# JohnLonginotto/uq

Hardware: NVIDIA B200
Metric: fastq_to_uq_encode_reads_per_s (higher is better)
Workload: dtype u8

## Files before the change

### uq_b200/csrc/common.cuh

```cuda
#pragma once
#include <cuda_runtime.h>
#include <stdint.h>
#include <stdio.h>
#include <string.h>
#include <string>
#include <vector>
#include <map>
#include "../../include/uqb200.h"

#define UQB_SM_COUNT 148

struct uqb_timer_rec { const char* name; cudaEvent_t a, b; uint64_t bytes; };
struct uqb_timer_tot { uint64_t launches = 0; double ms = 0; uint64_t bytes = 0; };

struct uqb_arena {
    unsigned long long base = 0;
    uint64_t reserved = 0;
    uint64_t mapped = 0;
    uint64_t granularity = 0;
    std::map<uint64_t, uint64_t> free_by_off;
    std::map<uint64_t, uint64_t> used;
    std::vector<unsigned long long> handles;
    std::vector<std::pair<uint64_t, uint64_t>> chunks;
};
// ... 106 lines not shown
static inline unsigned uqb_grid(uqb_ctx* ctx, uint64_t n, unsigned per_block, unsigned waves = 8) {
    uint64_t need = (n + per_block - 1) / per_block;
    uint64_t cap = (uint64_t)ctx->sm_count * waves;
    if (need < 1) need = 1;
    return (unsigned)(need < cap ? need : cap);
}

#ifdef __CUDACC__
__device__ __forceinline__ unsigned lane_id() { return threadIdx.x & 31u; }

__device__ __forceinline__ uint64_t load_be64(const uint8_t* p, uint32_t avail) {
    uint64_t v = 0;
#pragma unroll
    for (int i = 0; i < 8; i++) {
        uint64_t b = (uint32_t)i < avail ? (uint64_t)__ldg(p + i) : 0ull;
        v = (v << 8) | b;
    }
    return v;
}

__device__ __forceinline__ void atomic_min_i64(int64_t* addr, int64_t v) {
    atomicMin((long long*)addr, (long long)v);
}
__device__ __forceinline__ void atomic_max_i64(int64_t* addr, int64_t v) {
    atomicMax((long long*)addr, (long long)v);
}
#endif

#define UQB_SPLIT_TILE (256 * 64)
int uqb_split_count_tiles(uqb_ctx* ctx, const uint8_t* d, uint64_t n_end, uint64_t tile0, uint64_t ntiles, uint32_t* counts);
int uqb_split_write_tiles(uqb_ctx* ctx, const uint8_t* d, uint64_t n_end, uint64_t tile0, uint64_t ntiles, uint64_t line_base,
                          const uint64_t* bases, uint64_t* line_off);
int uqb_split_set_first(uqb_ctx* ctx, uint64_t* line_off);
int uqb_copy_stream(uqb_ctx* ctx, cudaStream_t* out);
int uqb_names_release(uqb_ctx* ctx, uqb_fastq* fq);

int uqb_scan_u32(uqb_ctx* ctx, const uint32_t* d_in, uint32_t* d_out, uint64_t n, uint32_t* d_total);
int uqb_scan_u32_to_u64(uqb_ctx* ctx, const uint32_t* d_in, uint64_t* d_out, uint64_t n, uint64_t* d_total);

struct uqb_sortbuf {
    uint64_t* key[2] = {nullptr, nullptr};
    uint32_t* aux[2] = {nullptr, nullptr};
    uint32_t* val[2] = {nullptr, nullptr};
    int cur = 0;
    uint64_t cap = 0;
};
int uqb_sortbuf_alloc(uqb_ctx* ctx, uqb_sortbuf* sb, uint64_t n, bool with_aux);
int uqb_sortbuf_free(uqb_ctx* ctx, uqb_sortbuf* sb);
int uqb_radix_sort(uqb_ctx* ctx, uqb_sortbuf* sb, uint64_t n, bool use_aux, const uint64_t* key_first = nullptr);
int uqb_scatter_pairs_u32(uqb_ctx* ctx, const uint32_t* idx, const uint32_t* val, uint64_t n, uint32_t* out);

int uqb_sort_rows_impl(uqb_ctx* ctx, const uint8_t* rows, uint64_t n, uint32_t width,
                       uint32_t** d_perm, uint32_t** d_gid_sorted, uint64_t* n_unique, const uint64_t* key0 = nullptr,
                       uint64_t** sorted_keys = nullptr);
```

### uq_b200/csrc/sort.cu

```cuda
#include "common.cuh"

#define ST 256

__global__ void __launch_bounds__(ST) k_chunk0_keys(const uint8_t* __restrict__ rows, uint64_t n, uint32_t width,
                                                   uint64_t* __restrict__ key, uint32_t* __restrict__ val) {
    uint64_t i = (uint64_t)blockIdx.x * ST + threadIdx.x;
    if (i >= n) return;
    key[i] = load_be64(rows + i * width, width < 8 ? width : 8);
    val[i] = (uint32_t)i;
}

#define SORT_ZOFF_MIN_WIDTH 256
__global__ void __launch_bounds__(ST) k_leading_zero_bytes(const uint8_t* __restrict__ rows, uint64_t n, uint32_t width,
                                                          uint32_t* __restrict__ zoff) {
    const unsigned lane = threadIdx.x & 31u;
    const uint64_t wstride = (uint64_t)gridDim.x * (ST / 32);
    for (uint64_t i = (uint64_t)blockIdx.x * (ST / 32) + (threadIdx.x >> 5); i < n; i += wstride) {
        const uint8_t* row = rows + i * width;
        uint32_t z = width;
        const uint32_t head = (uint32_t)((16u - ((uintptr_t)row & 15u)) & 15u);
        for (uint32_t b0 = 0; b0 < head && b0 < width && z == width; b0 += 32) {
            const uint32_t b = b0 + lane;
            const bool nz = b < head && b < width && row[b] != 0;
            const unsigned m = __ballot_sync(0xffffffffu, nz);
            if (m) z = b0 + (__ffs(m) - 1);
        }
        for (uint32_t b0 = head; b0 < width && z == width; b0 += 512) {
            const uint32_t b = b0 + lane * 16;
            uint32_t first = 16;
            if (b + 16 <= width) {
                const uint4 v = __ldg(reinterpret_cast<const uint4*>(row + b));
                if (v.x) first = (__ffs(v.x) - 1) >> 3;
                else if (v.y) first = 4 + ((__ffs(v.y) - 1) >> 3);
                else if (v.z) first = 8 + ((__ffs(v.z) - 1) >> 3);
                else if (v.w) first = 12 + ((__ffs(v.w) - 1) >> 3);
            } else if (b < width) {
                for (uint32_t k = 0; k < width - b; k++) if (row[b + k] != 0) { first = k; break; }
            }
            const unsigned m = __ballot_sync(0xffffffffu, first < 16);
            if (m) {
                const int src = __ffs(m) - 1;
                z = b0 + src * 16 + __shfl_sync(0xffffffffu, first, src);
            }
        }
        if (lane == 0) zoff[i] = z;
    }
}

__global__ void __launch_bounds__(ST) k_chunk0_keys_z(const uint8_t* __restrict__ rows, uint64_t n, uint32_t width, const uint32_t* __restrict__ zoff,
                                                     uint64_t* __restrict__ key, uint32_t* __restrict__ aux, uint32_t* __restrict__ val) {
    uint64_t i = (uint64_t)blockIdx.x * ST + threadIdx.x;
    if (i >= n) return;
    const uint32_t z = zoff[i], sig = width - z;
    key[i] = load_be64(rows + i * width + z, sig < 8 ? sig : 8);
    aux[i] = sig;
    val[i] = (uint32_t)i;
}

__global__ void __launch_bounds__(ST) k_mark_heads(const uint64_t* __restrict__ key, const uint32_t* __restrict__ aux, uint64_t n,
                                                  uint32_t* __restrict__ head) {
    uint64_t p = (uint64_t)blockIdx.x * ST + threadIdx.x;
    if (p >= n) return;
    head[p] = (p == 0 || key[p] != key[p - 1] || (aux && aux[p] != aux[p - 1])) ? 1u : 0u;
}

#define GLCP_EQUAL 0xFFFFFFFFu
__global__ void __launch_bounds__(ST) k_headpos(const uint32_t* __restrict__ head, const uint32_t* __restrict__ excl, uint64_t n,
                                               uint32_t* __restrict__ headpos, uint32_t* __restrict__ glcp) {
    uint64_t p = (uint64_t)blockIdx.x * ST + threadIdx.x;
    if (p >= n) return;
    if (head[p]) { headpos[excl[p]] = (uint32_t)p; glcp[excl[p]] = GLCP_EQUAL; }
    if (p == n - 1) headpos[excl[p] + head[p]] = (uint32_t)n;
}

template <int SUB>
__global__ void __launch_bounds__(ST) k_group_lcp(const uint8_t* __restrict__ rows, uint32_t width, uint32_t off, const uint32_t* __restrict__ zoff,
                                                 const uint32_t* __restrict__ perm, const uint32_t* __restrict__ head,
                                                 const uint32_t* __restrict__ excl, const uint32_t* __restrict__ headpos,
                                                 const uint8_t* __restrict__ done, uint64_t n, uint32_t* __restrict__ glcp) {
    constexpr uint32_t NP = 32u / SUB;
    constexpr int UN = 4;
    const unsigned lane = threadIdx.x & 31u, sg = lane / SUB, sl = lane % SUB;
    const uint64_t nblk = (n + 31) / 32, wstride = (uint64_t)gridDim.x * (ST / 32);
    for (uint64_t blk = (uint64_t)blockIdx.x * (ST / 32) + (threadIdx.x >> 5); blk < nblk; blk += wstride) {
        const uint64_t p = blk * 32 + lane;
        uint32_t ra = 0, rb = 0, g = 0, z = 0;
        bool live = false;
        if (p < n && !head[p] && !done[p]) {
            live = true;
            g = excl[p] - 1;
            ra = perm[p];
            rb = perm[headpos[g]];
            if (zoff) z = zoff[ra];
        }
        unsigned todo = __ballot_sync(0xffffffffu, live);
        if (!todo) continue;
        uint32_t mine = GLCP_EQUAL;
        for (uint32_t j0 = 0; j0 < 32; j0 += NP * UN) {
            if (!((todo >> j0) & ((NP * UN >= 32) ? 0xffffffffu : ((1u << (NP * UN)) - 1u)))) continue;
            uint32_t res[UN];
#pragma unroll
            for (int u = 0; u < UN; u++) res[u] = GLCP_EQUAL;
            uint32_t a_r[UN], b_r[UN], zz[UN];
            bool lv[UN];
#pragma unroll
            for (int u = 0; u < UN; u++) {
                const uint32_t j = j0 + u * NP + sg;
                a_r[u] = __shfl_sync(0xffffffffu, ra, j & 31u);
                b_r[u] = __shfl_sync(0xffffffffu, rb, j & 31u);
                zz[u] = __shfl_sync(0xffffffffu, z, j & 31u);
                lv[u] = j < 32u && ((todo >> (j & 31u)) & 1u);
            }
            const uint32_t maxrem = width - off;
            for (uint32_t w0 = 0; 4u * w0 < maxrem; w0 += SUB) {
                const uint32_t wd = w0 + sl;
                uint32_t xa[UN], xb[UN];
// ... 171 lines not shown
                        const uint32_t a = __shfl_sync(0xffffffffu, ord, pp & 31u);
                        int cc = 0;
#pragma unroll
                        for (int t = 0; t < TRIPS; t++) {
                            const uint32_t x = (pv && wvalid[t]) ? srows[a * pitch + t * SUB + sl] : y[t];
                            const unsigned ne = (__ballot_sync(0xffffffffu, x != y[t]) >> (sg * SUB)) & SUBMASK;
                            const unsigned lt = (__ballot_sync(0xffffffffu, x < y[t]) >> (sg * SUB)) & SUBMASK;
                            if (cc == 0 && ne) cc = ((lt >> (__ffs((int)ne) - 1)) & 1u) ? -1 : 1;
                        }
                        if (NP == 1) {
                            if (lane == q0) c = cc;
                        } else {
                            const int got = __shfl_sync(0xffffffffu, cc, ((lane - q0) * SUB) & 31u);
                            if (lane >= q0 && lane < q0 + NP && lane < hi) c = got;
                        }
                    }
                }
                have_c = false;
                const bool inr = lane >= lo && lane < hi;
                const unsigned less = __ballot_sync(0xffffffffu, inr && c < 0);
                const unsigned eq = __ballot_sync(0xffffffffu, inr && c == 0);
                const uint32_t nl = __popc(less), neq = __popc(eq);
                const uint32_t e0 = lo + nl, h0 = e0 + neq;
                if (nl | (hi - h0)) {
                    const unsigned gt = ((hi < 32u ? (1u << hi) : 0u) - (1u << lo)) & ~(less | eq);
                    uint32_t np = lane;
                    if (inr) np = c < 0 ? lo + __popc(less & ltm) : (c == 0 ? e0 + __popc(eq & ltm) : h0 + __popc(gt & ltm));
                    sord[np] = ord;
                    __syncwarp();
                    ord = sord[lane];
                    __syncwarp();
                }
                B |= 1u << e0;
                if (h0 < hi) B |= 1u << h0;
                R |= (uint32_t)((1ull << h0) - (1ull << e0));
                if (nl == 1u) R |= 1u << lo;
                if (hi - h0 == 1u) R |= 1u << h0;
            }
            const uint32_t rfin = __shfl_sync(0xffffffffu, r, ord & 31u);
            if (lane < sz) {
                perm[s + lane] = rfin;
                if (lane > 0) head[s + lane] = (B >> lane) & 1u;
                done[s + lane] = 1;
            }
            __syncwarp();
        }
    }
#pragma unroll
    for (int o = 16; o > 0; o >>= 1) my_large += __shfl_xor_sync(0xffffffffu, my_large, o);
    if (lane == 0 && my_large) atomicAdd(large_rows, my_large);
}

#define SGP_CHUNK 2048
template <int SUB>
__global__ void __launch_bounds__(ST) k_small_groups_packed(const uint8_t* __restrict__ rows, uint32_t width, uint32_t off,
                                                           uint32_t* __restrict__ perm, const uint32_t* __restrict__ head, uint32_t* __restrict__ head_out,
                                                           uint8_t* __restrict__ done, uint64_t n, uint32_t pitch,
                                                           unsigned long long* __restrict__ large_rows) {
    extern __shared__ uint32_t sg_smem[];
    constexpr uint32_t NP = 32u / SUB;
    constexpr uint32_t SUBMASK = SUB == 32 ? 0xffffffffu : ((1u << (SUB & 31)) - 1u);
    const unsigned lane = threadIdx.x & 31u, w = threadIdx.x >> 5;
    const unsigned sg = lane / SUB, sl = lane % SUB;
    uint32_t* srows = sg_smem + (size_t)w * (32 * pitch);
    const uint32_t rem = width - off;
    const bool wvalid = sl < pitch;
    const uint32_t nvalid = wvalid ? rem - 4u * sl : 0u;
    const uint32_t tailmask = nvalid >= 4u ? 0xffffffffu : (nvalid ? 0xffffffffu << ((4u - nvalid) * 8u) : 0u);
    const uint64_t nchunks = (n + SGP_CHUNK - 1) / SGP_CHUNK, warps_total = (uint64_t)gridDim.x * (ST / 32);
    unsigned long long my_large = 0;
    for (uint64_t ck = (uint64_t)blockIdx.x * (ST / 32) + w; ck < nchunks; ck += warps_total) {
        const uint64_t c0 = ck * SGP_CHUNK, c1 = (c0 + SGP_CHUNK < n) ? c0 + SGP_CHUNK : n;
        uint64_t cur = c0;
        while (cur < c1) {
            const unsigned hb = __ballot_sync(0xffffffffu, cur + lane < n ? head[cur + lane] != 0u : true);
            if (hb) { cur += (unsigned)__ffs((int)hb) - 1u; break; }
            cur += 32;
        }
        while (cur < c1) {
            const uint32_t r_spec = cur + lane < n ? perm[cur + lane] : 0u;
            const unsigned h1 = __ballot_sync(0xffffffffu, cur + lane < n ? head[cur + lane] != 0u : true);
            const unsigned h2 = __ballot_sync(0xffffffffu, cur + 32 + lane < n ? head[cur + 32 + lane] != 0u : true);
            const unsigned hi = (h1 >> 1) | (h2 << 31);
            if (!hi) {
                uint64_t nxt = c1;
                if (h2 >> 1) nxt = cur + 32 + ((unsigned)__ffs((int)(h2 >> 1)));
                else {
                    for (uint64_t q = cur + 64; q < c1; q += 32) {
                        const unsigned hb = __ballot_sync(0xffffffffu, q + lane < n ? head[q + lane] != 0u : true);
                        if (hb) { nxt = q + (unsigned)__ffs((int)hb) - 1u; break; }
                    }
                }
                if (lane == 0) my_large += 33;
                cur = nxt;
                continue;
            }
            const uint32_t cnt = 32u - (uint32_t)__clz((int)hi);
            const unsigned live = cnt == 32u ? 0xffffffffu : ((1u << cnt) - 1u);
            const unsigned hm = h1 & live;
            if (hm == live) { cur += cnt; continue; }
            const uint32_t r = lane < cnt ? r_spec : 0u;
            const unsigned upto = (2u << lane) - 1u;
            const uint32_t gs = 31u - (uint32_t)__clz((int)(hm & upto));
            const unsigned above = hm & ~upto;
            const uint32_t ge = above ? (uint32_t)__ffs((int)above) - 1u : cnt;
            const bool multi = lane < cnt && ge - gs > 1u;
            const unsigned need = __ballot_sync(0xffffffffu, multi);
#pragma unroll 4
            for (uint32_t j0 = 0; j0 < cnt; j0 += NP) {
                const uint32_t j = j0 + sg;
                const uint32_t rj = __shfl_sync(0xffffffffu, r, j & 31u);
                if (j < cnt && ((need >> j) & 1u) && wvalid) {
                    const uint64_t A = (uint64_t)(uintptr_t)rows + (uint64_t)rj * width + off;
                    const uint32_t ph = (uint32_t)A & 3u;
                    const uint32_t* base = reinterpret_cast<const uint32_t*>(A - ph) + sl;
                    const uint32_t lo = __ldg(base), hi2 = __ldg(base + 1);
                    srows[j * pitch + sl] = __byte_perm(__funnelshift_r(lo, hi2, ph * 8u), 0u, 0x0123) & tailmask;
                }
            }
            __syncwarp();
            const uint32_t maxsz = __reduce_max_sync(0xffffffffu, multi ? ge - gs : 0u);
            unsigned dmask = 0;
            for (uint32_t j0 = 0; j0 < cnt; j0 += NP) {
                const uint32_t j = j0 + sg;
                const uint32_t sj = __shfl_sync(0xffffffffu, gs, j & 31u);
                bool ne = false;
                if (j < cnt && ((need >> j) & 1u) && wvalid) ne = srows[j * pitch + sl] != srows[sj * pitch + sl];
                const unsigned b = __ballot_sync(0xffffffffu, ne);
#pragma unroll
                for (uint32_t s2 = 0; s2 < NP; s2++) if (lane == j0 + s2) dmask = (b >> (s2 * SUB)) & SUBMASK;
            }
            uint32_t rank = 0;
            bool eq_before = false;
            for (uint32_t t = 0; t < maxsz; t++) {
                const uint32_t i = gs + t;
                const bool act = multi && i < ge && i != lane;
                const unsigned di = __shfl_sync(0xffffffffu, dmask, act ? i : lane);
                if (act) {
                    unsigned m = di | dmask;
                    int c = 0;
                    while (m) {
                        const uint32_t wd = (uint32_t)__ffs((int)m) - 1u;
                        m &= m - 1u;
                        const uint32_t a = srows[i * pitch + wd], b = srows[lane * pitch + wd];
                        if (a != b) { c = a < b ? -1 : 1; break; }
                    }
                    if (c < 0 || (c == 0 && i < lane)) rank++;
                    if (c == 0 && i < lane) eq_before = true;
                }
            }
            __syncwarp();
            if (multi) {
                perm[cur + gs + rank] = r;
                if (rank > 0) head_out[cur + gs + rank] = eq_before ? 0u : 1u;
                done[cur + lane] = 1;
            }
            cur += cnt;
        }
    }
    if (lane == 0 && my_large) atomicAdd(large_rows, my_large);
}

__global__ void __launch_bounds__(ST) k_small_groups_gmem(const uint8_t* __restrict__ rows, uint32_t width, uint32_t off,
                                                         const uint32_t* __restrict__ zoff, uint32_t* __restrict__ perm, uint32_t* __restrict__ head, uint8_t* __restrict__ done,
                                                         const uint32_t* __restrict__ headpos, const uint32_t* __restrict__ d_ngroups,
                                                         unsigned long long* __restrict__ large_rows) {
    const unsigned lane = threadIdx.x & 31u, w = threadIdx.x >> 5;
    const uint32_t G = *d_ngroups;
    const uint64_t warps_total = (uint64_t)gridDim.x * (ST / 32);
    unsigned long long my_large = 0;
    for (uint64_t g0 = ((uint64_t)blockIdx.x * (ST / 32) + w) * 32; g0 < G; g0 += warps_total * 32) {
        const uint64_t g = g0 + lane;
        uint32_t start = 0, size = 0;
        if (g < G) { start = headpos[g]; size = headpos[g + 1] - start; }
        const bool fin = size < 2 || done[start];
        if (size > SG_MAX && !fin) my_large += size;
        unsigned need = __ballot_sync(0xffffffffu, size <= SG_MAX && !fin);
        while (need) {
            const int src = __ffs(need) - 1;
            need &= need - 1;
            const uint32_t s = __shfl_sync(0xffffffffu, start, src), sz = __shfl_sync(0xffffffffu, size, src);
            const uint32_t r = lane < sz ? perm[s + lane] : 0u;
            const uint32_t z = __shfl_sync(0xffffffffu, (zoff && lane < sz) ? zoff[r] : 0u, 0);
            const uint32_t rem = z + off < width ? width - z - off : 0u;
            uint32_t rank = 0;
            bool eq_before = false;
            for (uint32_t j = 0; j < sz; j++) {
                const uint32_t rj = __shfl_sync(0xffffffffu, r, j);
                if (lane < sz && j != lane) {
                    int c = 0;
                    const uint8_t* pa = rows + (uint64_t)rj * width + z + off;
                    const uint8_t* pb = rows + (uint64_t)r * width + z + off;
                    for (uint32_t i = 0; i < rem; i++) {
                        const unsigned a = __ldg(pa + i), b = __ldg(pb + i);
                        if (a != b) { c = a < b ? -1 : 1; break; }
                    }
                    if (c < 0 || (c == 0 && j < lane)) rank++;
                    if (c == 0 && j < lane) eq_before = true;
                }
            }
            __syncwarp();
            if (lane < sz) {
                perm[s + rank] = r;
                if (rank > 0) head[s + rank] = eq_before ? 0u : 1u;
                done[s + lane] = 1;
            }
            __syncwarp();
        }
    }
#pragma unroll
    for (int o = 16; o > 0; o >>= 1) my_large += __shfl_xor_sync(0xffffffffu, my_large, o);
    if (lane == 0 && my_large) atomicAdd(large_rows, my_large);
}

__global__ void __launch_bounds__(ST) k_compact_active(const uint8_t* __restrict__ rows, uint32_t width, const uint32_t* __restrict__ glcp,
                                                      const uint32_t* __restrict__ zoff, const uint32_t* __restrict__ act, const uint32_t* __restrict__ apos,
                                                      const uint32_t* __restrict__ head, const uint32_t* __restrict__ excl,
                                                      const uint32_t* __restrict__ perm, uint64_t n, uint32_t* __restrict__ pos_list,
                                                      uint64_t* __restrict__ key, uint32_t* __restrict__ aux, uint32_t* __restrict__ val) {
    uint64_t p = (uint64_t)blockIdx.x * ST + threadIdx.x;
    if (p >= n || !act[p]) return;
    uint32_t j = apos[p];
    uint32_t row = perm[p];
    pos_list[j] = (uint32_t)p;
    const uint32_t z = zoff ? zoff[row] : 0u;
    const uint32_t g = excl[p] + head[p] - 1;
    const uint32_t off = glcp[g];
    const uint32_t rem = z + off < width ? width - z - off : 0u;
    key[j] = load_be64(rows + (uint64_t)row * width + z + off, rem < 8 ? rem : 8);
    aux[j] = g;
    val[j] = row;
}

__global__ void __launch_bounds__(ST) k_write_back(const uint64_t* __restrict__ key, const uint32_t* __restrict__ aux,
                                                  const uint32_t* __restrict__ val, const uint32_t* __restrict__ pos_list, uint64_t m,
                                                  uint32_t* __restrict__ perm, uint32_t* __restrict__ head) {
    uint64_t j = (uint64_t)blockIdx.x * ST + threadIdx.x;
    if (j >= m) return;
    uint32_t p = pos_list[j];
    perm[p] = val[j];
    head[p] = (j == 0 || aux[j] != aux[j - 1] || key[j] != key[j - 1]) ? 1u : 0u;
}

__global__ void __launch_bounds__(ST) k_gid_from_scan(const uint32_t* __restrict__ head, uint32_t* __restrict__ excl_inout, uint64_t n) {
    uint64_t p = (uint64_t)blockIdx.x * ST + threadIdx.x;
    if (p >= n) return;
    excl_inout[p] = excl_inout[p] + head[p] - 1;
}

__global__ void __launch_bounds__(ST) k_iota_zero(uint32_t* __restrict__ perm, uint32_t* __restrict__ gid, uint64_t n) {
    uint64_t p = (uint64_t)blockIdx.x * ST + threadIdx.x;
    if (p >= n) return;
    perm[p] = (uint32_t)p;
    gid[p] = 0;
}

int uqb_sort_rows_impl(uqb_ctx* ctx, const uint8_t* rows, uint64_t n, uint32_t width,
                       uint32_t** d_perm, uint32_t** d_gid_sorted, uint64_t* n_unique, const uint64_t* key0, uint64_t** sorted_keys) {
    *d_perm = nullptr; *d_gid_sorted = nullptr; *n_unique = 0;
    if (sorted_keys) *sorted_keys = nullptr;
    if (n >= (1ull << 32)) return uqb_fail(ctx, "sort_rows: %llu rows exceed the 32-bit index range", (unsigned long long)n);
    uint32_t *perm = nullptr, *head, *excl;
    UQB_TRY(uqb_dalloc_t(ctx, &excl, n + 16));
    if (n == 0 || width == 0) UQB_TRY(uqb_dalloc_t(ctx, &perm, n + 16));
    if (n == 0) { *d_perm = perm; *d_gid_sorted = excl; return 0; }
    const unsigned nb = uqb_blocks(n, ST);
    if (width == 0) {
        UQB_LAUNCH(k_iota_zero, nb, ST, 0, perm, excl, n);
        *d_perm = perm; *d_gid_sorted = excl; *n_unique = 1;
        return 0;
    }
    UQB_TRY(uqb_dalloc_t(ctx, &head, n));
    uint32_t* d_tot;
    UQB_TRY(uqb_dalloc_t(ctx, &d_tot, 2));

    uint32_t* zoff = nullptr;
    if (width > SORT_ZOFF_MIN_WIDTH) {
        UQB_TRY(uqb_dalloc_t(ctx, &zoff, n));
        UQB_LAUNCH_B(n * 4, k_leading_zero_bytes, uqb_grid(ctx, n, ST / 32, 16), ST, 0, rows, n, width, zoff);
    }
    {
        uqb_sortbuf sb;
        UQB_TRY(uqb_sortbuf_alloc(ctx, &sb, n, zoff != nullptr));
        const uint64_t* kf = (!zoff && width >= 8) ? key0 : nullptr;
        if (zoff) UQB_LAUNCH_B(n * 24, k_chunk0_keys_z, nb, ST, 0, rows, n, width, zoff, sb.key[0], sb.aux[0], sb.val[0]);
        else if (!kf) UQB_LAUNCH_B(n * ((width < 8 ? width : 8) + 12), k_chunk0_keys, nb, ST, 0, rows, n, width, sb.key[0], sb.val[0]);
        UQB_TRY(uqb_radix_sort(ctx, &sb, n, zoff != nullptr, kf));
        UQB_LAUNCH(k_mark_heads, nb, ST, 0, sb.key[sb.cur], zoff ? sb.aux[sb.cur] : (const uint32_t*)nullptr, n, head);
        perm = sb.val[sb.cur];
        sb.val[sb.cur] = nullptr;
        if (sorted_keys && width <= 8 && !zoff) { *sorted_keys = sb.key[sb.cur]; sb.key[sb.cur] = nullptr; }
        UQB_TRY(uqb_sortbuf_free(ctx, &sb));
    }
    if (width > 8) {
        const uint32_t off = 8;
        uint32_t *headpos, *glcp, *act = nullptr, *apos = nullptr;
        uint8_t* done;
        unsigned long long* d_large;
        UQB_TRY(uqb_dalloc_t(ctx, &headpos, n + 1));
        UQB_TRY(uqb_dalloc_t(ctx, &glcp, n));
        UQB_TRY(uqb_dalloc_t(ctx, &done, n));
        UQB_TRY(uqb_dalloc_t(ctx, &d_large, 1));
        UQB_CUDA(cudaMemsetAsync(done, 0, n, ctx->stream));
        const uint32_t max_rounds = (width + 7) / 8 + 1;
        bool finished = false;
        if (width - off <= 128 && !zoff) {
            const uint32_t rem = width - off, pitch = (rem + 3) / 4;
            uint32_t* head2;
            UQB_TRY(uqb_dalloc_t(ctx, &head2, n));
            UQB_CUDA(cudaMemcpyAsync(head2, head, n * 4, cudaMemcpyDeviceToDevice, ctx->stream));
            UQB_CUDA(cudaMemsetAsync(d_large, 0, 8, ctx->stream));
            const size_t smem = (size_t)(ST / 32) * 32 * pitch * 4;
            const unsigned grid = uqb_grid(ctx, (n + SGP_CHUNK - 1) / SGP_CHUNK, ST / 32, 16);
            const uint64_t ab = n * ((uint64_t)rem + 13);
            if (pitch <= 8) {
                auto k_small_groups_packed_8 = k_small_groups_packed<8>;
                UQB_LAUNCH_B(ab, k_small_groups_packed_8, grid, ST, smem, rows, width, off, perm, head, head2, done, n, pitch, d_large);
            } else if (pitch <= 16) {
                auto k_small_groups_packed_16 = k_small_groups_packed<16>;
                UQB_LAUNCH_B(ab, k_small_groups_packed_16, grid, ST, smem, rows, width, off, perm, head, head2, done, n, pitch, d_large);
            } else {
                auto k_small_groups_packed_32 = k_small_groups_packed<32>;
                UQB_LAUNCH_B(ab, k_small_groups_packed_32, grid, ST, smem, rows, width, off, perm, head, head2, done, n, pitch, d_large);
            }
            UQB_TRY(uqb_dfree(ctx, head, n * 4));
            head = head2;
            unsigned long long large = 0;
            UQB_TRY(uqb_readback(ctx, &large, d_large, 8));
            finished = large == 0;
        }
        for (uint32_t round = 0; round < max_rounds && !finished; round++) {
            UQB_TRY(uqb_scan_u32(ctx, head, excl, n, d_tot));
            UQB_LAUNCH(k_headpos, nb, ST, 0, head, excl, n, headpos, glcp);
            const uint32_t rem = width - off;
            UQB_CUDA(cudaMemsetAsync(d_large, 0, 8, ctx->stream));
            const unsigned sg_grid = uqb_grid(ctx, n, ST, 16);
            if (rem <= SG_STAGE_BYTES && !zoff) {
                const uint32_t pitch = (rem + 3) / 4;
                const size_t smem = (size_t)(ST / 32) * (SG_MAX * pitch + 64) * 4;
                if (pitch <= 8) {
                    auto k_small_groups_8 = k_small_groups<8, 1>;
                    UQB_LAUNCH(k_small_groups_8, sg_grid, ST, smem, rows, width, off, perm, head, done, headpos, d_tot, pitch, d_large);
                } else if (pitch <= 16) {
                    auto k_small_groups_16 = k_small_groups<16, 1>;
                    UQB_LAUNCH(k_small_groups_16, sg_grid, ST, smem, rows, width, off, perm, head, done, headpos, d_tot, pitch, d_large);
                } else if (pitch <= 32) {
                    auto k_small_groups_32 = k_small_groups<32, 1>;
                    UQB_CUDA(cudaFuncSetAttribute(k_small_groups_32, cudaFuncAttributeMaxDynamicSharedMemorySize, (int)smem));
                    UQB_LAUNCH(k_small_groups_32, sg_grid, ST, smem, rows, width, off, perm, head, done, headpos, d_tot, pitch, d_large);
                } else {
                    auto k_small_groups_64 = k_small_groups<32, 2>;
                    UQB_CUDA(cudaFuncSetAttribute(k_small_groups_64, cudaFuncAttributeMaxDynamicSharedMemorySize, (int)smem));
                    UQB_LAUNCH(k_small_groups_64, sg_grid, ST, smem, rows, width, off, perm, head, done, headpos, d_tot, pitch, d_large);
                }
            } else {
                UQB_LAUNCH(k_small_groups_gmem, sg_grid, ST, 0, rows, width, off, zoff, perm, head, done, headpos, d_tot, d_large);
            }
            unsigned long long large = 0;
            UQB_TRY(uqb_readback(ctx, &large, d_large, 8));
            if (large == 0) break;
            const uint64_t ab_lcp = n * ((uint64_t)rem + 16);
            if (rem <= 32) {
                auto k_group_lcp_8 = k_group_lcp<8>;
                UQB_LAUNCH_B(ab_lcp, k_group_lcp_8, uqb_grid(ctx, n, ST, 16), ST, 0, rows, width, off, zoff, perm, head, excl, headpos, done, n, glcp);
            } else {
                auto k_group_lcp_32 = k_group_lcp<32>;
                UQB_LAUNCH_B(ab_lcp, k_group_lcp_32, uqb_grid(ctx, n, ST, 16), ST, 0, rows, width, off, zoff, perm, head, excl, headpos, done, n, glcp);
            }
            if (!act) {
                UQB_TRY(uqb_dalloc_t(ctx, &act, n));
                UQB_TRY(uqb_dalloc_t(ctx, &apos, n));
            }
            UQB_LAUNCH(k_active_flags, nb, ST, 0, head, excl, glcp, done, n, act);
            UQB_TRY(uqb_scan_u32(ctx, act, apos, n, d_tot + 1));
            uint32_t tot[2];
            UQB_TRY(uqb_readback(ctx, tot, d_tot, 8));
            const uint64_t m = tot[1];
            if (m == 0) break;
            uqb_sortbuf sb;
            uint32_t* pos_list;
            UQB_TRY(uqb_sortbuf_alloc(ctx, &sb, m, true));
            UQB_TRY(uqb_dalloc_t(ctx, &pos_list, m));
            UQB_LAUNCH_B(n * 8 + m * 32, k_compact_active, nb, ST, 0, rows, width, glcp, zoff, act, apos, head, excl, perm, n, pos_list, sb.key[0], sb.aux[0], sb.val[0]);
            UQB_TRY(uqb_radix_sort(ctx, &sb, m, true));
            UQB_LAUNCH_B(m * 28, k_write_back, uqb_blocks(m, ST), ST, 0, sb.key[sb.cur], sb.aux[sb.cur], sb.val[sb.cur], pos_list, m, perm, head);
            UQB_TRY(uqb_dfree(ctx, pos_list, m * 4));
            UQB_TRY(uqb_sortbuf_free(ctx, &sb));
        }
        UQB_TRY(uqb_dfree(ctx, headpos, (n + 1) * 4));
        UQB_TRY(uqb_dfree(ctx, glcp, n * 4));
        if (act) { UQB_TRY(uqb_dfree(ctx, act, n * 4)); UQB_TRY(uqb_dfree(ctx, apos, n * 4)); }
        UQB_TRY(uqb_dfree(ctx, done, n));
        UQB_TRY(uqb_dfree(ctx, d_large, 8));
    }
    if (zoff) UQB_TRY(uqb_dfree(ctx, zoff, n * 4));
    UQB_TRY(uqb_scan_u32(ctx, head, excl, n, d_tot));
    UQB_LAUNCH(k_gid_from_scan, nb, ST, 0, head, excl, n);
    uint32_t u;
    UQB_TRY(uqb_readback(ctx, &u, d_tot, 4));
    UQB_TRY(uqb_dfree(ctx, d_tot, 8));
    UQB_TRY(uqb_dfree(ctx, head, n * 4));
    *d_perm = perm;
    *d_gid_sorted = excl;
    *n_unique = u;
    return 0;
}

__global__ void __launch_bounds__(ST) k_scatter_key(const uint32_t* __restrict__ perm, const uint32_t* __restrict__ gid, uint64_t n,
                                                   uint32_t* __restrict__ key) {
    uint64_t p = (uint64_t)blockIdx.x * ST + threadIdx.x;
    if (p >= n) return;
    key[perm[p]] = gid[p];
}

static int scatter_key(uqb_ctx* ctx, const uint32_t* perm, const uint32_t* gid, uint64_t n, uint32_t* key) {
    if (n == 0) return 0;
    const uint32_t wshift = 23;
    if (n <= (3ull << wshift)) {
        UQB_LAUNCH_B(n * 12, k_scatter_key, uqb_blocks(n, ST), ST, 0, perm, gid, n, key);
        return 0;
    }
    return uqb_scatter_pairs_u32(ctx, perm, gid, n, key);
}

__global__ void __launch_bounds__(ST) k_first_of_group(const uint32_t* __restrict__ perm, const uint32_t* __restrict__ gid, uint64_t n,
                                                      uint32_t* __restrict__ first_row) {
    uint64_t p = (uint64_t)blockIdx.x * ST + threadIdx.x;
    if (p >= n) return;
    if (p == 0 || gid[p] != gid[p - 1]) first_row[gid[p]] = perm[p];
}

__global__ void __launch_bounds__(ST) k_uniq_from_keys(const uint64_t* __restrict__ skey, const uint32_t* __restrict__ gid, uint64_t n,
                                                      uint32_t width, uint8_t* __restrict__ out) {
    for (uint64_t p = (uint64_t)blockIdx.x * ST + threadIdx.x; p < n; p += (uint64_t)gridDim.x * ST) {
        const uint32_t g = gid[p];
        if (p && gid[p - 1] == g) continue;
        const uint64_t k = skey[p];
        uint8_t* o = out + (uint64_t)g * width;
        for (uint32_t b = 0; b < width; b++) o[b] = (uint8_t)(k >> (56 - 8 * b));
    }
}

__global__ void __launch_bounds__(ST) k_gather_rows(const uint8_t* __restrict__ table, uint32_t width, const uint32_t* __restrict__ idx,
                                                   uint64_t nrows, uint8_t* __restrict__ out) {
    const unsigned lane = threadIdx.x & 31u;
    const uint64_t wstride = (uint64_t)gridDim.x * (ST / 32);
    for (uint64_t i = (uint64_t)blockIdx.x * (ST / 32) + (threadIdx.x >> 5); i < nrows; i += wstride) {
        const uint8_t* src = table + (uint64_t)__ldg(idx + i) * width;
        uint8_t* dst = out + i * width;
        for (uint32_t b = lane; b < width; b += 32) dst[b] = __ldg(src + b);
    }
}
// ... 44 lines not shown
    __shared__ __align__(16) uint8_t stage[ST * 16];
    const uint64_t nblk = (nrows + ST - 1) / ST;
    for (uint64_t blk = blockIdx.x; blk < nblk; blk += gridDim.x) {
        const uint64_t i0 = blk * ST, i = i0 + threadIdx.x;
        const uint32_t nr = (uint32_t)(nrows - i0 < ST ? nrows - i0 : ST);
        __syncthreads();
        if (i < nrows) {
            const uint8_t* s = table + (uint64_t)__ldg(idx + i) * width;
            for (uint32_t b = 0; b < width; b++) stage[threadIdx.x * width + b] = __ldg(s + b);
        }
        __syncthreads();
        const uint32_t total = nr * width;
        uint8_t* dst = out + i0 * width;
        for (uint32_t k = threadIdx.x; k < (total >> 2); k += ST) reinterpret_cast<uint32_t*>(dst)[k] = reinterpret_cast<const uint32_t*>(stage)[k];
        if (threadIdx.x < (total & 3u)) dst[(total & ~3u) + threadIdx.x] = stage[(total & ~3u) + threadIdx.x];
    }
}

template <typename T>
__global__ void __launch_bounds__(ST) k_gather_items(const T* __restrict__ table, const uint32_t* __restrict__ idx, uint64_t n, T* __restrict__ out) {
    for (uint64_t i = (uint64_t)blockIdx.x * ST + threadIdx.x; i < n; i += (uint64_t)gridDim.x * ST) out[i] = table[idx[i]];
}

static int gather_rows_impl(uqb_ctx* ctx, const void* table, uint32_t width, const uint32_t* idx, uint64_t n, void* out) {
    if (n == 0 || width == 0) return 0;
    const uint64_t ab = n * (2 * (uint64_t)width + 4);
    const unsigned g = uqb_grid(ctx, n, ST, 16);
    switch (width) {
        case 1: UQB_LAUNCH_B(ab, k_gather_items<uint8_t>, g, ST, 0, (const uint8_t*)table, idx, n, (uint8_t*)out); return 0;
        case 2: UQB_LAUNCH_B(ab, k_gather_items<uint16_t>, g, ST, 0, (const uint16_t*)table, idx, n, (uint16_t*)out); return 0;
        case 4: UQB_LAUNCH_B(ab, k_gather_items<uint32_t>, g, ST, 0, (const uint32_t*)table, idx, n, (uint32_t*)out); return 0;
        case 8: UQB_LAUNCH_B(ab, k_gather_items<uint64_t>, g, ST, 0, (const uint64_t*)table, idx, n, (uint64_t*)out); return 0;
    }
    if ((reinterpret_cast<uintptr_t>(out) & 3u) == 0) {
        if (width <= 16) {
            UQB_LAUNCH_B(ab, k_gather_narrow, uqb_grid(ctx, n, ST, 16), ST, 0, (const uint8_t*)table, width, idx, n, (uint8_t*)out);
            return 0;
        }
        if (width <= GR_MAXW) {
            UQB_LAUNCH_B(ab, k_gather_rows32, uqb_grid(ctx, n, ST, 16), ST, 0, (const uint8_t*)table, width, 128u / width, 128u % width, idx, n, (uint8_t*)out);
            return 0;
        }
    }
    UQB_LAUNCH_B(ab, k_gather_rows, uqb_grid(ctx, n, ST / 32, 16), ST, 0, (const uint8_t*)table, width, idx, n, (uint8_t*)out);
    return 0;
}

extern "C" int uqb_sort_rows(uqb_ctx* ctx, const uqb_array* table, uqb_array** perm, uqb_array** key,
                             uqb_array** key_sorted, uqb_array** uniq, uint64_t* n_unique) {
    uint32_t *d_perm, *d_gid;
    uint64_t u = 0;
    const uint64_t n = table->n;
    uint64_t* skeys = nullptr;
    UQB_TRY(uqb_sort_rows_impl(ctx, (const uint8_t*)table->d, n, table->width, &d_perm, &d_gid, &u, table->key0, uniq ? &skeys : nullptr));
    if (n_unique) *n_unique = u;
    const unsigned nb = uqb_blocks(n, ST);
    if (key) {
        UQB_TRY(uqb_new_array(ctx, n, 4, key));
        UQB_TRY(scatter_key(ctx, d_perm, d_gid, n, (uint32_t*)(*key)->d));
    }
    if (uniq) {
        UQB_TRY(uqb_new_array(ctx, u, table->width, uniq));
        if (skeys) {
            UQB_LAUNCH_B(n * 12 + u * table->width, k_uniq_from_keys, uqb_grid(ctx, n, ST, 16), ST, 0, skeys, d_gid, n, table->width, (uint8_t*)(*uniq)->d);
            UQB_TRY(uqb_dfree(ctx, skeys, n * 8));
        } else if (n && table->width) {
            uint32_t* first_row;
            UQB_TRY(uqb_dalloc_t(ctx, &first_row, u));
            UQB_LAUNCH(k_first_of_group, nb, ST, 0, d_perm, d_gid, n, first_row);
            UQB_TRY(gather_rows_impl(ctx, table->d, table->width, first_row, u, (*uniq)->d));
            UQB_TRY(uqb_dfree(ctx, first_row, u * 4));
        }
    }
    if (key_sorted) UQB_TRY(uqb_adopt_array(ctx, d_gid, n, 4, key_sorted));
    else UQB_TRY(uqb_dfree(ctx, d_gid, n * 4));
    if (perm) UQB_TRY(uqb_adopt_array(ctx, d_perm, n, 4, perm));
    else UQB_TRY(uqb_dfree(ctx, d_perm, n * 4));
    return 0;
}

extern "C" int uqb_gather_rows(uqb_ctx* ctx, const uqb_array* table, const uqb_array* perm, uqb_array** out) {
    if (perm->width != 4) return uqb_fail(ctx, "gather_rows: index array must be uint32");
    UQB_TRY(uqb_new_array(ctx, perm->n, table->width, out));
    UQB_TRY(gather_rows_impl(ctx, table->d, table->width, (const uint32_t*)perm->d, perm->n, (*out)->d));
    return 0;
}

template <typename T>
__global__ void __launch_bounds__(ST) k_narrow(const uint32_t* __restrict__ in, uint64_t n, T* __restrict__ out) {
    for (uint64_t i = (uint64_t)blockIdx.x * ST + threadIdx.x; i < n; i += (uint64_t)gridDim.x * ST) out[i] = (T)in[i];
}

extern "C" int uqb_narrow_u32(uqb_ctx* ctx, const uqb_array* a, uint32_t itemsize, uqb_array** out) {
    if (a->width != 4) return uqb_fail(ctx, "narrow: input must be uint32");
    UQB_TRY(uqb_new_array(ctx, a->n, itemsize, out));
    if (a->n == 0) return 0;
    unsigned g = uqb_grid(ctx, a->n, ST, 16);
    const uint32_t* in = (const uint32_t*)a->d;
    switch (itemsize) {
        case 1: UQB_LAUNCH(k_narrow<uint8_t>, g, ST, 0, in, a->n, (uint8_t*)(*out)->d); break;
        case 2: UQB_LAUNCH(k_narrow<uint16_t>, g, ST, 0, in, a->n, (uint16_t*)(*out)->d); break;
        case 4: UQB_LAUNCH(k_narrow<uint32_t>, g, ST, 0, in, a->n, (uint32_t*)(*out)->d); break;
        case 8: UQB_LAUNCH(k_narrow<uint64_t>, g, ST, 0, in, a->n, (uint64_t*)(*out)->d); break;
        default: return uqb_fail(ctx, "narrow: itemsize %u", itemsize);
    }
    return 0;
}

template <typename T>
__global__ void __launch_bounds__(ST) k_index_u32(const T* __restrict__ in, uint64_t n, uint64_t bound, uint32_t* __restrict__ out,
                                                 unsigned long long* __restrict__ first_bad) {
    unsigned long long bad = ~0ull;
    for (uint64_t i = (uint64_t)blockIdx.x * ST + threadIdx.x; i < n; i += (uint64_t)gridDim.x * ST) {
        const unsigned long long v = (unsigned long long)in[i];
// ... 368 lines not shown
```

Before: 775.9 million.

## Emit unique rows directly from the small-group finisher kernel into per-chunk slots

When unique rows are requested and width fits, the small-group sort finisher writes each distinct row (sorted key prefix plus staged tail bytes) into per-chunk slots. A prefix scan then compacts them into the output, replacing the separate first-of-group plus gather-rows pass. It also adds a group-count readback after head marking, which gates the path on duplication being at least two to one. The cost is extra shared memory, lower occupancy bounds, a slot buffer sized to n·width, and an added host sync.

```diff
diff --git a/uq_b200/csrc/common.cuh b/uq_b200/csrc/common.cuh
--- a/uq_b200/csrc/common.cuh
+++ b/uq_b200/csrc/common.cuh
@@ -182,4 +182,4 @@
 
 int uqb_sort_rows_impl(uqb_ctx* ctx, const uint8_t* rows, uint64_t n, uint32_t width,
                        uint32_t** d_perm, uint32_t** d_gid_sorted, uint64_t* n_unique, const uint64_t* key0 = nullptr,
-                       uint64_t** sorted_keys = nullptr);
+                       uint64_t** sorted_keys = nullptr, uqb_array** uniq = nullptr);
diff --git a/uq_b200/csrc/sort.cu b/uq_b200/csrc/sort.cu
--- a/uq_b200/csrc/sort.cu
+++ b/uq_b200/csrc/sort.cu
@@ -58,10 +58,14 @@
 }
 
 __global__ void __launch_bounds__(ST) k_mark_heads(const uint64_t* __restrict__ key, const uint32_t* __restrict__ aux, uint64_t n,
-                                                  uint32_t* __restrict__ head) {
+                                                  uint32_t* __restrict__ head, uint32_t* __restrict__ ngroups) {
     uint64_t p = (uint64_t)blockIdx.x * ST + threadIdx.x;
-    if (p >= n) return;
-    head[p] = (p == 0 || key[p] != key[p - 1] || (aux && aux[p] != aux[p - 1])) ? 1u : 0u;
+    const bool h = p < n && (p == 0 || key[p] != key[p - 1] || (aux && aux[p] != aux[p - 1]));
+    if (p < n) head[p] = h ? 1u : 0u;
+    if (ngroups) {
+        const unsigned b = __ballot_sync(0xffffffffu, h);
+        if ((threadIdx.x & 31u) == 0 && b) atomicAdd(ngroups, (uint32_t)__popc(b));
+    }
 }
 
 #define GLCP_EQUAL 0xFFFFFFFFu
@@ -339,26 +343,34 @@
 }
 
 #define SGP_CHUNK 2048
-template <int SUB>
-__global__ void __launch_bounds__(ST) k_small_groups_packed(const uint8_t* __restrict__ rows, uint32_t width, uint32_t off,
-                                                           uint32_t* __restrict__ perm, const uint32_t* __restrict__ head, uint32_t* __restrict__ head_out,
-                                                           uint8_t* __restrict__ done, uint64_t n, uint32_t pitch,
-                                                           unsigned long long* __restrict__ large_rows) {
+#define SGP_SLOT (SGP_CHUNK + 32)
+template <int SUB, bool EMIT>
+__device__ __forceinline__ void small_groups_packed(const uint8_t* __restrict__ rows, uint32_t width, uint32_t off,
+                                                    uint32_t* __restrict__ perm, const uint32_t* __restrict__ head, uint32_t* __restrict__ head_out,
+                                                    uint8_t* __restrict__ done, uint64_t n, uint32_t pitch,
+                                                    unsigned long long* __restrict__ large_rows, const uint64_t* __restrict__ skey,
+                                                    uint8_t* __restrict__ slots, uint32_t* __restrict__ slot_rows) {
     extern __shared__ uint32_t sg_smem[];
     constexpr uint32_t NP = 32u / SUB;
     constexpr uint32_t SUBMASK = SUB == 32 ? 0xffffffffu : ((1u << (SUB & 31)) - 1u);
+    constexpr uint32_t KW = EMIT ? 2u : 0u;
     const unsigned lane = threadIdx.x & 31u, w = threadIdx.x >> 5;
     const unsigned sg = lane / SUB, sl = lane % SUB;
-    uint32_t* srows = sg_smem + (size_t)w * (32 * pitch);
+    const uint32_t stride = pitch + KW;
+    uint32_t* const srows0 = sg_smem + (size_t)w * (32 * stride + (EMIT ? 32 : 0));
+    uint32_t* const srows = srows0 + KW;
+    uint32_t* const smap = srows0 + 32 * stride;
     const uint32_t rem = width - off;
     const bool wvalid = sl < pitch;
     const uint32_t nvalid = wvalid ? rem - 4u * sl : 0u;
     const uint32_t tailmask = nvalid >= 4u ? 0xffffffffu : (nvalid ? 0xffffffffu << ((4u - nvalid) * 8u) : 0u);
     const uint64_t nchunks = (n + SGP_CHUNK - 1) / SGP_CHUNK, warps_total = (uint64_t)gridDim.x * (ST / 32);
+    const float inv_w = 1.0f / (float)width;
     unsigned long long my_large = 0;
     for (uint64_t ck = (uint64_t)blockIdx.x * (ST / 32) + w; ck < nchunks; ck += warps_total) {
         const uint64_t c0 = ck * SGP_CHUNK, c1 = (c0 + SGP_CHUNK < n) ? c0 + SGP_CHUNK : n;
         uint64_t cur = c0;
+        uint32_t nd = 0;
         while (cur < c1) {
             const unsigned hb = __ballot_sync(0xffffffffu, cur + lane < n ? head[cur + lane] != 0u : true);
             if (hb) { cur += (unsigned)__ffs((int)hb) - 1u; break; }
@@ -366,6 +378,7 @@
         }
         while (cur < c1) {
             const uint32_t r_spec = cur + lane < n ? perm[cur + lane] : 0u;
+            const uint64_t k_spec = EMIT && cur + lane < n ? skey[cur + lane] : 0ull;
             const unsigned h1 = __ballot_sync(0xffffffffu, cur + lane < n ? head[cur + lane] != 0u : true);
             const unsigned h2 = __ballot_sync(0xffffffffu, cur + 32 + lane < n ? head[cur + 32 + lane] != 0u : true);
             const unsigned hi = (h1 >> 1) | (h2 << 31);
@@ -382,10 +395,14 @@
                 cur = nxt;
                 continue;
             }
-            const uint32_t cnt = 32u - (uint32_t)__clz((int)hi);
+            uint32_t cnt = 32u - (uint32_t)__clz((int)hi);
+            if (EMIT && c1 - cur <= 32u) {
+                const unsigned nxt = hi >> (uint32_t)(c1 - cur - 1);
+                if (nxt) cnt = min(cnt, (uint32_t)(c1 - cur) + (uint32_t)__ffs((int)nxt) - 1u);
+            }
             const unsigned live = cnt == 32u ? 0xffffffffu : ((1u << cnt) - 1u);
             const unsigned hm = h1 & live;
-            if (hm == live) { cur += cnt; continue; }
+            if (!EMIT && hm == live) { cur += cnt; continue; }
             const uint32_t r = lane < cnt ? r_spec : 0u;
             const unsigned upto = (2u << lane) - 1u;
             const uint32_t gs = 31u - (uint32_t)__clz((int)(hm & upto));
@@ -393,16 +410,17 @@
             const uint32_t ge = above ? (uint32_t)__ffs((int)above) - 1u : cnt;
             const bool multi = lane < cnt && ge - gs > 1u;
             const unsigned need = __ballot_sync(0xffffffffu, multi);
+            if (EMIT && lane < cnt) { srows0[lane * stride] = (uint32_t)(k_spec >> 32); srows0[lane * stride + 1] = (uint32_t)k_spec; }
 #pragma unroll 4
             for (uint32_t j0 = 0; j0 < cnt; j0 += NP) {
                 const uint32_t j = j0 + sg;
                 const uint32_t rj = __shfl_sync(0xffffffffu, r, j & 31u);
-                if (j < cnt && ((need >> j) & 1u) && wvalid) {
+                if (j < cnt && (EMIT || ((need >> j) & 1u)) && wvalid) {
                     const uint64_t A = (uint64_t)(uintptr_t)rows + (uint64_t)rj * width + off;
                     const uint32_t ph = (uint32_t)A & 3u;
                     const uint32_t* base = reinterpret_cast<const uint32_t*>(A - ph) + sl;
                     const uint32_t lo = __ldg(base), hi2 = __ldg(base + 1);
-                    srows[j * pitch + sl] = __byte_perm(__funnelshift_r(lo, hi2, ph * 8u), 0u, 0x0123) & tailmask;
+                    srows[j * stride + sl] = __byte_perm(__funnelshift_r(lo, hi2, ph * 8u), 0u, 0x0123) & tailmask;
                 }
             }
             __syncwarp();
@@ -412,7 +430,7 @@
                 const uint32_t j = j0 + sg;
                 const uint32_t sj = __shfl_sync(0xffffffffu, gs, j & 31u);
                 bool ne = false;
-                if (j < cnt && ((need >> j) & 1u) && wvalid) ne = srows[j * pitch + sl] != srows[sj * pitch + sl];
+                if (j < cnt && ((need >> j) & 1u) && wvalid) ne = srows[j * stride + sl] != srows[sj * stride + sl];
                 const unsigned b = __ballot_sync(0xffffffffu, ne);
 #pragma unroll
                 for (uint32_t s2 = 0; s2 < NP; s2++) if (lane == j0 + s2) dmask = (b >> (s2 * SUB)) & SUBMASK;
@@ -429,7 +447,7 @@
                     while (m) {
                         const uint32_t wd = (uint32_t)__ffs((int)m) - 1u;
                         m &= m - 1u;
-                        const uint32_t a = srows[i * pitch + wd], b = srows[lane * pitch + wd];
+                        const uint32_t a = srows[i * stride + wd], b = srows[lane * stride + wd];
                         if (a != b) { c = a < b ? -1 : 1; break; }
                     }
                     if (c < 0 || (c == 0 && i < lane)) rank++;
@@ -442,10 +460,95 @@
                 if (rank > 0) head_out[cur + gs + rank] = eq_before ? 0u : 1u;
                 done[cur + lane] = 1;
             }
+            if (EMIT) {
+                const uint32_t fp = multi ? gs + rank : lane;
+                const bool dist = lane < cnt && !eq_before;
+                const unsigned dbits = __reduce_or_sync(0xffffffffu, dist ? 1u << fp : 0u);
+                if (dist) smap[__popc(dbits & ((1u << fp) - 1u))] = lane;
+                __syncwarp();
+                const uint32_t total = (uint32_t)__popc(dbits) * width;
+                const uint64_t b0 = (uint64_t)nd * width;
+                uint8_t* const slot = slots + ck * (uint64_t)SGP_SLOT * width;
+                const uint32_t lead = (uint32_t)b0 & 3u;
+                uint32_t* const wdst = reinterpret_cast<uint32_t*>(slot + (b0 - lead));
+                for (uint32_t k = lane; 4u * k < lead + total; k += 32) {
+                    const int e = (int)(4u * k) - (int)lead;
+                    if (e >= 0 && (uint32_t)e + 4u <= total) {
+                        uint32_t rr = (uint32_t)__float2uint_rz((float)e * inv_w), c = (uint32_t)e - rr * width;
+                        if (c >= width) { c -= width; rr++; }
+                        const uint32_t* sr = srows0 + smap[rr] * stride;
+                        uint32_t v = __funnelshift_r(__byte_perm(sr[c >> 2], 0u, 0x0123), __byte_perm(sr[(c >> 2) + 1], 0u, 0x0123), (c & 3u) * 8u);
+                        if (c + 4u > width) {
+                            const uint32_t n0 = width - c;
+                            const uint32_t* sr2 = srows0 + smap[rr + 1] * stride;
+                            v = (v & (0xffffffffu >> (8u * (4u - n0)))) | (__byte_perm(sr2[0], 0u, 0x0123) << (8u * n0));
+                        }
+                        wdst[k] = v;
+                    } else {
+                        for (int b = 0; b < 4; b++) {
+                            const int x = e + b;
+                            if (x < 0 || (uint32_t)x >= total) continue;
+                            const uint32_t rr = (uint32_t)x / width, c = (uint32_t)x - rr * width;
+                            const uint32_t v = srows0[smap[rr] * stride + (c >> 2)];
+                            slot[b0 + (uint32_t)x] = (uint8_t)(v >> (24u - 8u * (c & 3u)));
+                        }
+                    }
+                }
+                nd += (uint32_t)__popc(dbits);
+                __syncwarp();
+            }
             cur += cnt;
         }
+        if (EMIT && lane == 0) slot_rows[ck] = nd;
     }
     if (lane == 0 && my_large) atomicAdd(large_rows, my_large);
+}
+
+template <int SUB>
+__global__ void __launch_bounds__(ST) k_small_groups_packed(const uint8_t* __restrict__ rows, uint32_t width, uint32_t off,
+                                                           uint32_t* __restrict__ perm, const uint32_t* __restrict__ head, uint32_t* __restrict__ head_out,
+                                                           uint8_t* __restrict__ done, uint64_t n, uint32_t pitch,
+                                                           unsigned long long* __restrict__ large_rows) {
+    small_groups_packed<SUB, false>(rows, width, off, perm, head, head_out, done, n, pitch, large_rows, nullptr, nullptr, nullptr);
+}
+
+template <int SUB>
+__global__ void __launch_bounds__(ST, SUB == 32 ? 6 : 5) k_small_groups_packed_emit(const uint8_t* __restrict__ rows, uint32_t width, uint32_t off,
+                                                           uint32_t* __restrict__ perm, const uint32_t* __restrict__ head, uint32_t* __restrict__ head_out,
+                                                           uint8_t* __restrict__ done, uint64_t n, uint32_t pitch,
+                                                           unsigned long long* __restrict__ large_rows, const uint64_t* __restrict__ skey,
+                                                           uint8_t* __restrict__ slots, uint32_t* __restrict__ slot_rows) {
+    small_groups_packed<SUB, true>(rows, width, off, perm, head, head_out, done, n, pitch, large_rows, skey, slots, slot_rows);
+}
+
+__global__ void __launch_bounds__(ST) k_pack_slots(const uint8_t* __restrict__ slots, uint32_t width, const uint32_t* __restrict__ slot_rows,
+                                                  const uint32_t* __restrict__ pre, uint64_t nslots, uint8_t* __restrict__ out) {
+    for (uint64_t ck = blockIdx.x; ck < nslots; ck += gridDim.x) {
+        const uint8_t* src = slots + ck * (uint64_t)SGP_SLOT * width;
+        uint8_t* dst = out + (uint64_t)pre[ck] * width;
+        const uint32_t len = slot_rows[ck] * width;
+        const uint32_t head = (uint32_t)((16u - ((uintptr_t)dst & 15u)) & 15u);
+        const uint32_t body = len > head ? (len - head) & ~15u : 0u;
+        for (uint32_t b = threadIdx.x; b < len; b += ST)
+            if (b < head || b >= head + body) dst[b] = src[b];
+        const uint32_t q = head >> 2, sh = (head & 3u) * 8u;
+        for (uint32_t k = threadIdx.x; 16u * k < body; k += ST) {
+            const uint4 a = __ldg(reinterpret_cast<const uint4*>(src) + k), b = __ldg(reinterpret_cast<const uint4*>(src) + k + 1);
+            uint32_t x[5];
+            switch (q) {
+                case 0: x[0] = a.x; x[1] = a.y; x[2] = a.z; x[3] = a.w; x[4] = b.x; break;
+                case 1: x[0] = a.y; x[1] = a.z; x[2] = a.w; x[3] = b.x; x[4] = b.y; break;
+                case 2: x[0] = a.z; x[1] = a.w; x[2] = b.x; x[3] = b.y; x[4] = b.z; break;
+                default: x[0] = a.w; x[1] = b.x; x[2] = b.y; x[3] = b.z; x[4] = b.w; break;
+            }
+            uint4 v;
+            v.x = __funnelshift_r(x[0], x[1], sh);
+            v.y = __funnelshift_r(x[1], x[2], sh);
+            v.z = __funnelshift_r(x[2], x[3], sh);
+            v.w = __funnelshift_r(x[3], x[4], sh);
+            *reinterpret_cast<uint4*>(dst + head + 16u * k) = v;
+        }
+    }
 }
 
 __global__ void __launch_bounds__(ST) k_small_groups_gmem(const uint8_t* __restrict__ rows, uint32_t width, uint32_t off,
@@ -543,9 +646,11 @@
 }
 
 int uqb_sort_rows_impl(uqb_ctx* ctx, const uint8_t* rows, uint64_t n, uint32_t width,
-                       uint32_t** d_perm, uint32_t** d_gid_sorted, uint64_t* n_unique, const uint64_t* key0, uint64_t** sorted_keys) {
+                       uint32_t** d_perm, uint32_t** d_gid_sorted, uint64_t* n_unique, const uint64_t* key0, uint64_t** sorted_keys,
+                       uqb_array** uniq) {
     *d_perm = nullptr; *d_gid_sorted = nullptr; *n_unique = 0;
     if (sorted_keys) *sorted_keys = nullptr;
+    if (uniq) *uniq = nullptr;
     if (n >= (1ull << 32)) return uqb_fail(ctx, "sort_rows: %llu rows exceed the 32-bit index range", (unsigned long long)n);
     uint32_t *perm = nullptr, *head, *excl;
     UQB_TRY(uqb_dalloc_t(ctx, &excl, n + 16));
@@ -561,6 +666,8 @@
     uint32_t* d_tot;
     UQB_TRY(uqb_dalloc_t(ctx, &d_tot, 2));
 
+    const bool emit_fit = uniq && width > 8 && width - 8 <= 128;
+    uint64_t* skey = nullptr;
     uint32_t* zoff = nullptr;
     if (width > SORT_ZOFF_MIN_WIDTH) {
         UQB_TRY(uqb_dalloc_t(ctx, &zoff, n));
@@ -573,12 +680,22 @@
         if (zoff) UQB_LAUNCH_B(n * 24, k_chunk0_keys_z, nb, ST, 0, rows, n, width, zoff, sb.key[0], sb.aux[0], sb.val[0]);
         else if (!kf) UQB_LAUNCH_B(n * ((width < 8 ? width : 8) + 12), k_chunk0_keys, nb, ST, 0, rows, n, width, sb.key[0], sb.val[0]);
         UQB_TRY(uqb_radix_sort(ctx, &sb, n, zoff != nullptr, kf));
-        UQB_LAUNCH(k_mark_heads, nb, ST, 0, sb.key[sb.cur], zoff ? sb.aux[sb.cur] : (const uint32_t*)nullptr, n, head);
+        if (emit_fit) UQB_CUDA(cudaMemsetAsync(d_tot, 0, 4, ctx->stream));
+        UQB_LAUNCH(k_mark_heads, nb, ST, 0, sb.key[sb.cur], zoff ? sb.aux[sb.cur] : (const uint32_t*)nullptr, n, head,
+                   emit_fit ? d_tot : (uint32_t*)nullptr);
         perm = sb.val[sb.cur];
         sb.val[sb.cur] = nullptr;
+        if (emit_fit) {
+            uint32_t groups = 0;
+            UQB_TRY(uqb_readback(ctx, &groups, d_tot, 4));
+            if (2 * (uint64_t)groups <= n) { skey = sb.key[sb.cur]; sb.key[sb.cur] = nullptr; }
+        }
         if (sorted_keys && width <= 8 && !zoff) { *sorted_keys = sb.key[sb.cur]; sb.key[sb.cur] = nullptr; }
         UQB_TRY(uqb_sortbuf_free(ctx, &sb));
     }
+    const uint64_t nslots = (n + SGP_CHUNK - 1) / SGP_CHUNK;
+    uint8_t* slots = nullptr;
+    uint32_t *slot_rows = nullptr, *slot_pre = nullptr;
     if (width > 8) {
         const uint32_t off = 8;
         uint32_t *headpos, *glcp, *act = nullptr, *apos = nullptr;
@@ -597,24 +714,51 @@
             UQB_TRY(uqb_dalloc_t(ctx, &head2, n));
             UQB_CUDA(cudaMemcpyAsync(head2, head, n * 4, cudaMemcpyDeviceToDevice, ctx->stream));
             UQB_CUDA(cudaMemsetAsync(d_large, 0, 8, ctx->stream));
-            const size_t smem = (size_t)(ST / 32) * 32 * pitch * 4;
-            const unsigned grid = uqb_grid(ctx, (n + SGP_CHUNK - 1) / SGP_CHUNK, ST / 32, 16);
-            const uint64_t ab = n * ((uint64_t)rem + 13);
-            if (pitch <= 8) {
-                auto k_small_groups_packed_8 = k_small_groups_packed<8>;
-                UQB_LAUNCH_B(ab, k_small_groups_packed_8, grid, ST, smem, rows, width, off, perm, head, head2, done, n, pitch, d_large);
-            } else if (pitch <= 16) {
-                auto k_small_groups_packed_16 = k_small_groups_packed<16>;
-                UQB_LAUNCH_B(ab, k_small_groups_packed_16, grid, ST, smem, rows, width, off, perm, head, head2, done, n, pitch, d_large);
+            const unsigned grid = uqb_grid(ctx, nslots, ST / 32, 16);
+            if (!skey) {
+                const size_t smem = (size_t)(ST / 32) * 32 * pitch * 4;
+                const uint64_t ab = n * ((uint64_t)rem + 13);
+                if (pitch <= 8) {
+                    auto k_small_groups_packed_8 = k_small_groups_packed<8>;
+                    UQB_LAUNCH_B(ab, k_small_groups_packed_8, grid, ST, smem, rows, width, off, perm, head, head2, done, n, pitch, d_large);
+                } else if (pitch <= 16) {
+                    auto k_small_groups_packed_16 = k_small_groups_packed<16>;
+                    UQB_LAUNCH_B(ab, k_small_groups_packed_16, grid, ST, smem, rows, width, off, perm, head, head2, done, n, pitch, d_large);
+                } else {
+                    auto k_small_groups_packed_32 = k_small_groups_packed<32>;
+                    UQB_LAUNCH_B(ab, k_small_groups_packed_32, grid, ST, smem, rows, width, off, perm, head, head2, done, n, pitch, d_large);
+                }
             } else {
-                auto k_small_groups_packed_32 = k_small_groups_packed<32>;
-                UQB_LAUNCH_B(ab, k_small_groups_packed_32, grid, ST, smem, rows, width, off, perm, head, head2, done, n, pitch, d_large);
+                UQB_TRY(uqb_dalloc_t(ctx, &slots, nslots * SGP_SLOT * width + 16));
+                UQB_TRY(uqb_dalloc_t(ctx, &slot_rows, nslots));
+                const size_t smem = (size_t)(ST / 32) * (32 * (pitch + 2) + 32) * 4;
+                const uint64_t ab = n * ((uint64_t)width + 25);
+                if (pitch <= 8) {
+                    auto k_small_groups_packed_emit_8 = k_small_groups_packed_emit<8>;
+                    UQB_LAUNCH_B(ab, k_small_groups_packed_emit_8, grid, ST, smem, rows, width, off, perm, head, head2, done, n, pitch, d_large,
+                                 skey, slots, slot_rows);
+                } else if (pitch <= 16) {
+                    auto k_small_groups_packed_emit_16 = k_small_groups_packed_emit<16>;
+                    UQB_LAUNCH_B(ab, k_small_groups_packed_emit_16, grid, ST, smem, rows, width, off, perm, head, head2, done, n, pitch, d_large,
+                                 skey, slots, slot_rows);
+                } else {
+                    auto k_small_groups_packed_emit_32 = k_small_groups_packed_emit<32>;
+                    UQB_LAUNCH_B(ab, k_small_groups_packed_emit_32, grid, ST, smem, rows, width, off, perm, head, head2, done, n, pitch, d_large,
+                                 skey, slots, slot_rows);
+                }
+                UQB_TRY(uqb_dfree(ctx, skey, n * 8));
+                skey = nullptr;
             }
             UQB_TRY(uqb_dfree(ctx, head, n * 4));
             head = head2;
             unsigned long long large = 0;
             UQB_TRY(uqb_readback(ctx, &large, d_large, 8));
             finished = large == 0;
+            if (slots && !finished) {
+                UQB_TRY(uqb_dfree(ctx, slots, nslots * SGP_SLOT * width + 16));
+                UQB_TRY(uqb_dfree(ctx, slot_rows, nslots * 4));
+                slots = nullptr; slot_rows = nullptr;
+            }
         }
         for (uint32_t round = 0; round < max_rounds && !finished; round++) {
             UQB_TRY(uqb_scan_u32(ctx, head, excl, n, d_tot));
@@ -683,8 +827,23 @@
     if (zoff) UQB_TRY(uqb_dfree(ctx, zoff, n * 4));
     UQB_TRY(uqb_scan_u32(ctx, head, excl, n, d_tot));
     UQB_LAUNCH(k_gid_from_scan, nb, ST, 0, head, excl, n);
-    uint32_t u;
-    UQB_TRY(uqb_readback(ctx, &u, d_tot, 4));
+    if (slots) {
+        UQB_TRY(uqb_dalloc_t(ctx, &slot_pre, nslots));
+        UQB_TRY(uqb_scan_u32(ctx, slot_rows, slot_pre, nslots, d_tot + 1));
+    }
+    uint32_t tot[2] = {0, 0};
+    UQB_TRY(uqb_readback(ctx, tot, d_tot, slots ? 8 : 4));
+    const uint32_t u = tot[0];
+    if (slots) {
+        if (tot[1] != u)
+            return uqb_fail(ctx, "sort_rows: the finisher emitted %u distinct rows, the group heads count %u", tot[1], u);
+        UQB_TRY(uqb_new_array(ctx, u, width, uniq));
+        UQB_LAUNCH_B(2ull * u * width, k_pack_slots, uqb_grid(ctx, nslots, 1, 16), ST, 0, slots, width, slot_rows, slot_pre, nslots,
+                     (uint8_t*)(*uniq)->d);
+        UQB_TRY(uqb_dfree(ctx, slots, nslots * SGP_SLOT * width + 16));
+        UQB_TRY(uqb_dfree(ctx, slot_rows, nslots * 4));
+        UQB_TRY(uqb_dfree(ctx, slot_pre, nslots * 4));
+    }
     UQB_TRY(uqb_dfree(ctx, d_tot, 8));
     UQB_TRY(uqb_dfree(ctx, head, n * 4));
     *d_perm = perm;
@@ -835,14 +994,18 @@
     uint64_t u = 0;
     const uint64_t n = table->n;
     uint64_t* skeys = nullptr;
-    UQB_TRY(uqb_sort_rows_impl(ctx, (const uint8_t*)table->d, n, table->width, &d_perm, &d_gid, &u, table->key0, uniq ? &skeys : nullptr));
+    uqb_array* emitted = nullptr;
+    UQB_TRY(uqb_sort_rows_impl(ctx, (const uint8_t*)table->d, n, table->width, &d_perm, &d_gid, &u, table->key0, uniq ? &skeys : nullptr,
+                               uniq ? &emitted : nullptr));
     if (n_unique) *n_unique = u;
     const unsigned nb = uqb_blocks(n, ST);
     if (key) {
         UQB_TRY(uqb_new_array(ctx, n, 4, key));
         UQB_TRY(scatter_key(ctx, d_perm, d_gid, n, (uint32_t*)(*key)->d));
     }
-    if (uniq) {
+    if (uniq && emitted) {
+        *uniq = emitted;
+    } else if (uniq) {
         UQB_TRY(uqb_new_array(ctx, u, table->width, uniq));
         if (skeys) {
             UQB_LAUNCH_B(n * 12 + u * table->width, k_uniq_from_keys, uqb_grid(ctx, n, ST, 16), ST, 0, skeys, d_gid, n, table->width, (uint8_t*)(*uniq)->d);
```

Result: slower. 734.4 million, median of 6 (-5.3%).
